# nomadkaraoke/python-audio-separator

Measured on AMD Instinct MI355X. Metric: audio-sec separated / wall-sec (RTF), UVR-MDX-NET 44.1kHz stereo, 1/2/4/8 GPU, higher is better.
Workload: dtype f32 (I/O and accumulators; matrix products on the 16-bit pipe from block-scaled two-part fp16 operands, 22-bit products -- see arithmetic; fp32-exact setting timed in arithmetic_ab)

## Files before the change

### python-audio-separator_amd/csrc/asx.hip

```cpp
#include <hip/hip_runtime.h>

#include <algorithm>
#include <atomic>
#include <cmath>
#include <cstdarg>
#include <cstdio>
#include <cstdlib>
#include <cstring>
#include <functional>
#include <map>
#include <string>
#include <mutex>
#include <vector>

#include "../../include/asx.h"
#include "knobs.h"
#include "resample_plan.h"

static void grant_lds(const void *kernel, int bytes) {
  static std::mutex mu;
  static std::map<const void *, int> granted;
  std::lock_guard<std::mutex> lock(mu);
  int &g = granted[kernel];
  if (bytes > g) {
// ... 31 lines not shown
#include "engine_mdx.h"

static int opt_nonneg(int32_t v) { return v < 0 ? 0 : (int)v; }
static int opt_onoff(int32_t v) { return v > 0 ? 1 : 0; }

static const struct EngineOption {
  const char *key;
  int asx_engine::*field;
  int EngineKnobs::*knob;
  int (*norm)(int32_t);
  const char *refusal = nullptr;
  int shipped = 0;
} kOptions[] = {
    {"winograd", &asx_engine::winograd, &EngineKnobs::winograd, opt_nonneg,
     "asx_set_option: winograd = %d names a superseded kernel generation that only an experimental build carries "
     "(python build.py --experimental); this library has 0 (direct kernel) and 3 (the default)", 3},
    {"winograd_stationary", &asx_engine::winos, &EngineKnobs::winos, opt_nonneg,
     "asx_set_option: the weight-stationary Winograd kernel (measured slower) is in experimental builds only (python build.py --experimental)"},
    {"winograd_bf16x6", &asx_engine::wino6, &EngineKnobs::wino6, opt_nonneg},
    {"gemm_bf16x6", &asx_engine::gemm_bf16x6, &EngineKnobs::gemm_bf16x6, opt_onoff},
    {"gemm_f16x3", &asx_engine::gemm_f16x3, &EngineKnobs::gemm_f16x3, opt_onoff},
    {"conv_direct_f16x3", &asx_engine::conv3h, &EngineKnobs::conv3h, opt_nonneg},
    {"conv_fuse_input", &asx_engine::conv_fuse_input, &EngineKnobs::conv_fuse_input, opt_onoff},
    {"conv_down_bf16x6", &asx_engine::down6, &EngineKnobs::down6, opt_onoff},
    {"conv_up_bf16x6", &asx_engine::up6, &EngineKnobs::up6, opt_onoff},
    {"gemm_pair_images", &asx_engine::pair_images, &EngineKnobs::pair_images, opt_onoff,
     "asx_set_option: gemm_pair_images = 1 needs an experimental build (python build.py --experimental): the pair-image reader measured no "
     "faster in the nets and is not in the default library"},
};

static const EngineOption *find_option(const char *fn, const char *key) {
  for (const EngineOption &o : kOptions)
    if (!strcmp(key, o.key)) return &o;
  set_err("%s: unknown option '%s'", fn, key);
  return nullptr;
}

extern "C" {

int asx_abi_version(void) { return ASX_ABI_VERSION; }
const char *asx_last_error(void) { return g_err; }

int asx_device_count(void) {
  int n = 0;
  if (hipGetDeviceCount(&n) != hipSuccess) return 0;
  return n;
// ... 163 lines not shown
  e->sinc_tab.release();
  for (RsTable *t : e->rs_tabs) {
    t->tab.release();
    delete t;
  }
  e->rs_tabs.clear();
  e->d_window.release();
  e->d_tw.release();
  e->d_env.release();
  e->d_tw3.release();
  e->d_hann3.release();
  e->seam3.release();
  e->d_zeros.release();
  free_conv(e->first);
  free_conv(e->final_);
  for (auto &b : e->enc) free_block(b);
  for (auto &b : e->dec) free_block(b);
  free_block(e->mid);
  for (auto &c : e->ds) free_conv(c);
  for (auto &c : e->us) free_conv(c);
  e->spec_in.release();
  e->spec_out.release();
  for (auto &r : e->R) r.release();
  e->H.release();
  e->frames.release();
  e->chunk_out.release();
  e->d_starts.release();
  e->d_nact.release();
  e->d_peak.release();
  e->d_demixed.release();
  e->d_div.release();
  for (DevBuf *b : {&e->pool_wave, &e->pool_nsong, &e->pool_songs, &e->pool_div, &e->pool_peak}) b->release();
  for (auto &sk : e->skip) sk.release();
  if (e->v3) v3_destroy(e->v3);
  if (e->rof) rof_destroy(e->rof);
  hd_drop_clones(e);
  if (e->ht) ht_destroy(e->ht);
  if (e->hd) hd_destroy(e->hd);
  if (e->vr) vr_destroy(e->vr);
  if (e->ens) ens_destroy(e->ens);
  delete e;
}

int asx_net_begin(asx_engine *e, const asx_net_config *cfg) {
  w3_flush(e);
  REQUIRE(e && cfg, "asx_net_begin: null argument");
// ... 912 lines not shown
    kind = CK_DOWN;
    to = t / 2;
    fo = f / 2;
  } else if (!strcmp(op, "conv1x1")) kind = CK_1X1;
  else if (!strcmp(op, "up")) {
    kind = CK_UP;
    to = 2 * t;
    fo = 2 * f;
    REQUIRE(aux_host, "asx_op_conv(up): skip tensor required");
  } else {
    set_err("asx_op_conv: unknown op '%s'", op);
    return ASX_ERR_INVALID;
  }
  ConvLayer L;
  DevBuf dx, dy, dskip;
  BufGuard g{{&dx, &dy, &dskip, &L.w, &L.b, &L.wu, &L.wu2, &L.wu3, &L.wus, &L.wu6, &L.wu6h, &L.w3h, &L.wd6, &L.wup6}};
  CHK(conv_setup(L, kind, cin, cout, relu ? 1 : 0));
  CHK(conv_pack(L, w_host, b_host, e->winograd));
  CHK(to_dev(dx, x_host, (size_t)B * cin * t * f));
  const size_t ny = (size_t)B * cout * to * fo;
  CHK(dy.ensure(ny * 4));
  HIPCHK(hipMemset(dy.p, 0xff, ny * 4));
  if (kind == CK_UP) CHK(to_dev(dskip, aux_host, ny));
  CHK(conv_launch(e, L, dx.f(), dskip.f(), dy.f(), B, t, f, nullptr));
  CHK(to_host(y_host, dy, ny));
  return ASX_OK;
}

int asx_op_tdf(asx_engine *e, const float *x_host, int32_t B, int32_t c, int32_t t, int32_t k, const float *w_host,
               const float *bias_host, int32_t n, const float *scale_host, const float *shift_host,
               const float *res_host, float *y_host) {
  REQUIRE(e && x_host && w_host && scale_host && shift_host && y_host && B > 0 && c > 0 && t > 0 && k > 0 && n > 0,
          "asx_op_tdf: bad argument");
  HIPCHK(hipSetDevice(e->device));
  TdfLayer L;
  DevBuf dx, dy, dres;
  BufGuard g{{&dx, &dy, &dres, &L.w, &L.bias, &L.scale, &L.shift}};
  CHK(tdf_pack(L, n, k, c, w_host, bias_host, scale_host, shift_host));
  const int64_t M = (int64_t)B * c * t;
  CHK(to_dev(dx, x_host, (size_t)M * k));
  CHK(dy.ensure((size_t)M * n * 4));
  HIPCHK(hipMemset(dy.p, 0xff, (size_t)M * n * 4));
  if (res_host) CHK(to_dev(dres, res_host, (size_t)M * n));
  const int rc = tdf_launch(e, L, dx.f(), res_host ? dres.f() : nullptr, dy.f(), M, t, nullptr);
  const int rc2 = rc == ASX_OK ? to_host(y_host, dy, (size_t)M * n) : rc;
  w3_drop(e, L.w.p);
// ... 1258 lines not shown
```

### python-audio-separator_amd/csrc/engine_core.h

```cpp
#pragma once

static thread_local char g_err[512] = "";
static void set_err(const char *fmt, ...) {
  va_list ap;
  va_start(ap, fmt);
  vsnprintf(g_err, sizeof(g_err), fmt, ap);
  va_end(ap);
}
#define HIPCHK(x)                                                                       \
  do {                                                                                  \
    hipError_t e_ = (x);                                                                \
    if (e_ != hipSuccess) {                                                             \
      set_err("%s:%d %s -> %s", __FILE__, __LINE__, #x, hipGetErrorString(e_));         \
      return ASX_ERR_HIP;                                                               \
    }                                                                                   \
  } while (0)
#define CHK(x)                    \
  do {                            \
    int r_ = (x);                 \
    if (r_ != ASX_OK) return r_;  \
  } while (0)
#define REQUIRE(cond, ...)        \
  do {                            \
    if (!(cond)) {                \
// ... 143 lines not shown
  std::vector<HdNet *> hd_cl;
  DevBuf hd_lstm_ws;
  VrNet *vr = nullptr;
  EnsCtx *ens = nullptr;
  asx_mdx_config cfg{};
  FftPlan plan{};
  DevBuf d_window, d_tw, d_env;
  std::vector<float> custom_window;
  DevBuf d_hann3;
  DevBuf d_tw3, seam3;
  bool fft3 = false;
  bool fft3p = false;
  DevBuf d_zeros;
  bool net_begun = false, net_ready = false;
  asx_net_config net{};
  std::map<std::string, std::vector<float>> host_tensors;
  ConvLayer first, final_;
  std::vector<Block> enc, dec;
  Block mid;
  std::vector<ConvLayer> ds, us;
  int ws_batch = 0;
  DevBuf spec_in, spec_out, R[3], H, HE, frames, chunk_out, d_starts, d_nact, d_peak, d_demixed;
  DevBuf pool_wave, pool_nsong, pool_songs, pool_div, pool_peak;
  DevBuf gn_part;
  DevBuf d_div;
  DivKey div_key;
  DevBuf sinc_tab;
  std::vector<RsTable *> rs_tabs;
  std::mutex rs_mu;
  hipEvent_t div_ev = nullptr;
  hipStream_t div_stream = nullptr;
  std::vector<DevBuf> skip;
  int winograd = 3;
  int winos = 0;
  int gemm_bf16x6 = 1;
  int gemm_f16x3 = 1;
  int wino6 = 144;
  int conv3h = 144;
  int conv_fuse_input = 1;
  int down6 = 1;
  int up6 = 1;
  int pair_images = 0;
  std::vector<W3Entry> w3;
  std::mutex w3_mu;
  bool prof = false;
  int prof_nprod = 0;
  std::vector<ProfRec> recs;
};

static int pick_batch(const asx_engine *e) { return e->cfg.max_batch > 0 ? e->cfg.max_batch : 64; }

#include "batching.h"

template <class F>
static int timed(asx_engine *e, int cls, double flops, double bytes, hipStream_t s, F &&launch) {
  if (!e->prof) {
    launch();
    HIPCHK(hipGetLastError());
    return ASX_OK;
  }
  ProfRec r;
// ... 66 lines not shown
```

### python-audio-separator_amd/csrc/engine_mdx.h

```cpp
#pragma once

template <class CFG>
static void launch_conv_t(const ConvArgs &a, int nblk, hipStream_t s) {
  grant_lds(&conv_mfma_kernel<CFG>, CFG::LDS_BYTES);
  hipLaunchKernelGGL(conv_mfma_kernel<CFG>, dim3(nblk), dim3(256), CFG::LDS_BYTES, s, a);
}

static int conv_tile_h(int kind) { return kind == CK_UP ? 4 : 8; }

static int pick_nrep_conv(int cout) {
  const int ct = (cout + 15) / 16;
  int best = 1, best_pad = 1 << 30;
  for (int n = 3; n >= 1; --n) {
    const int pad = ((ct + n - 1) / n) * n - ct;
    if (pad < best_pad) {
      best_pad = pad;
      best = n;
    }
  }
  return best;
}
static int pick_nrep_up(int cout) {
  const int ct = (cout + 15) / 16;
  if (knobs().up_nrep == 4 && (4 * ct) % 4 == 0) return 4;
// ... 194 lines not shown
static std::atomic<long long> g_down6_launches{0};
static std::atomic<long long> g_up6_launches{0};

struct ConvView {
  int64_t x_bstride = 0;
  int64_t y_bstride = 0;
  const float *res = nullptr;
  int64_t aux_bstride = 0;
  int act = -1;
  float alpha = 1.f;
  const ConvLayer *fin = nullptr;
  const float *fin_x = nullptr;
};

static bool conv3h_takes(const asx_engine *e, const ConvLayer &L, bool dma, const float *res, int act, int T, int F, int64_t y_bstride, const float *y) {
#ifdef ASX_EXPERIMENTAL_KERNELS
  if (e->winos == 1 && L.wus.p != nullptr) return false;
#endif
  return L.kind == CK_3X3 && e->winograd == 3 && e->gemm_bf16x6 > 0 && e->gemm_f16x3 > 0 && e->conv3h > 0 && L.cin <= e->conv3h && L.w3h.p != nullptr && dma &&
         res == nullptr && (act == ACT_RELU || act == ACT_NONE) && F % 32 == 0 && (int64_t)Conv3hCfg::C * T * F < ((int64_t)1 << 29) &&
         y_bstride % 4 == 0 && (reinterpret_cast<uintptr_t>(y) & 15) == 0;
}

static int conv_launch(asx_engine *e, const ConvLayer &L, const float *x, const float *skip, float *y, int B, int T,
                       int F, hipStream_t s, const ConvView &v = ConvView()) {
  ConvArgs a{};
  a.x = x;
  a.wp = L.w.f();
  a.bias = L.b.f();
  a.skip = skip;
  a.res = v.res;
  a.zeros = e->d_zeros.f();
  a.y = y;
  a.B = B;
  a.Cin = L.cin;
  a.Cout = L.cout;
  a.T = T;
  a.F = F;
  a.act = v.act >= 0 ? v.act : (L.relu ? ACT_RELU : ACT_NONE);
  a.alpha = v.alpha;
  REQUIRE(a.act != ACT_ELU || L.kind == CK_1X1, "ELU epilogue: 1x1 convolutions only");
  a.CG = L.cg;
  a.NCI = L.nci;
  a.nt = knobs().nt & 1;
  int cls = ASX_PROF_CONV3X3;
  double taps = 9;
// ... 70 lines not shown
    if (ragged) return k12 ? gos(&conv_winos_kernel<12, 0, true>, WinoSCfg<12>::LDS_BYTES) : gos(&conv_winos_kernel<24, 0, true>, WinoSCfg<24>::LDS_BYTES);
    return k12 ? gos(&conv_winos_kernel<12, 0, false>, WinoSCfg<12>::LDS_BYTES) : gos(&conv_winos_kernel<24, 0, false>, WinoSCfg<24>::LDS_BYTES);
  }
#endif
  if (conv3h_takes(e, L, dma, v.res, a.act, T, F, a.y_bstride, y)) {
    const int nb = L.cin / Conv3hCfg::C;
    const int tilesT = (T + 3) / 4, tilesF = F / 32;
    int bw = 32;
    double best = 1e30;
    for (int cand : {32, 16, 8}) {
      if ((tilesT * cand) % 32 != 0) continue;
      const int tps = tilesT * cand / 32;
      const int bands = (tilesF + cand - 1) / cand, items = B * bands;
      const double cost = (double)(bands * cand) / tilesF * (tps + 1.0) / tps * (double)((items + 7) / 8) / (items / 8.0);
      if (cost < best - 1e-9) {
        best = cost;
        bw = cand;
      }
    }
    if (best > 1e29) bw = 32;
    grant_lds(&conv3h_kernel<0, false>, Conv3hCfg::LDS_BYTES);
    grant_lds(&conv3h_kernel<0, true>, Conv3hCfg::LDS_BYTES);
    grant_lds(&conv3h_kernel<0, false, true>, Conv3hCfg::LDS_BYTES);
    const int64_t plane = (int64_t)T * F;
    return timed(e, cls, flops, bytes, s, [&]() {
      e->prof_nprod = 3;
      for (int ob = 0; ob < nb; ++ob)
        for (int ib = 0; ib < nb; ++ib) {
          Conv3hArgs ca{};
          ca.x = x + (int64_t)ib * Conv3hCfg::C * plane;
          ca.y = y + (int64_t)ob * Conv3hCfg::C * plane;
          ca.prev = ib > 0 ? ca.y : nullptr;
          ca.wimg = reinterpret_cast<const u32x4 *>(reinterpret_cast<const uint32_t *>(L.w3h.p) + (size_t)(ob * nb + ib) * Conv3hCfg::IMG_U32);
          ca.bias = ib == 0 ? L.b.f() + ob * Conv3hCfg::C : nullptr;
          ca.B = B;
          ca.T = T;
          ca.F = F;
          ca.x_bstride = a.x_bstride;
          ca.y_bstride = a.y_bstride;
          ca.act = ib == nb - 1 ? a.act : ACT_NONE;
          ca.tilesT = tilesT;
          ca.tilesF = tilesF;
          ca.bw = bw;
          ca.tps = (tilesT * bw) % 32 == 0 ? tilesT * bw / 32 : tilesT;
          if (v.fin) {
            ca.xin = v.fin_x;
            ca.xin_bstride = 4 * plane;
            ca.w1 = v.fin->w1f.f();
            hipLaunchKernelGGL((conv3h_kernel<0, false, true>), dim3(256), dim3(512), Conv3hCfg::LDS_BYTES, s, ca);
            g_conv3h_fin_launches.fetch_add(1);
          } else if (ib > 0) hipLaunchKernelGGL((conv3h_kernel<0, true>), dim3(256), dim3(512), Conv3hCfg::LDS_BYTES, s, ca);
          else hipLaunchKernelGGL((conv3h_kernel<0, false>), dim3(256), dim3(512), Conv3hCfg::LDS_BYTES, s, ca);
          g_conv3h_launches.fetch_add(1);
        }
    });
  }
  if (L.kind == CK_3X3 && e->winograd == 3 && e->gemm_bf16x6 > 0 && e->wino6 > 0 && L.cin >= e->wino6 && dma && L.wu6_nci > 0 &&
      (int64_t)T * F < ((int64_t)1 << 24)) {
    ConvArgs wa = a;
    const bool h3 = e->gemm_f16x3 > 0 && L.wu6h.p != nullptr;
    wa.wp = reinterpret_cast<const float *>(h3 ? L.wu6h.p : L.wu6.p);
    wa.CG = L.wu_cg;
    wa.NCI = L.wu6_nci;
    wa.tilesT = (a.To + Wino6Cfg::TH - 1) / Wino6Cfg::TH;
    wa.tilesF = (a.Fo + Wino6Cfg::TW - 1) / Wino6Cfg::TW;
    const int64_t S = (int64_t)wa.tilesT * wa.tilesF * B;
    const int64_t nb = ((S + 7) / 8) * 8 * wa.CG;
    if (nb < ((int64_t)1 << 31)) {
      grant_lds(&conv_wino6_kernel<0, 1>, Wino6Cfg::LDS_BYTES);
      grant_lds(&conv_wino6_kernel<0, 1, true>, Wino6Cfg::LDS_BYTES);
      g_wino6_launches.fetch_add(1);
      if (h3) g_wino6h_launches.fetch_add(1);
      return timed(e, cls, flops, bytes, s, [&]() {
        e->prof_nprod = h3 ? 3 : 6;
// ... 776 lines not shown
  CHK(conv_launch(e, e->final_, cur, nullptr, spec_out, B, T, F, s));
  return ASX_OK;
}

static int ensure_workspace(asx_engine *e, int Bchunks, bool need_net) {
  const int T = e->cfg.segment_size, Fq = e->cfg.dim_f;
  const int mult = (need_net && e->cfg.enable_denoise) ? 2 : 1;
  const size_t Bn = (size_t)Bchunks * mult;
  CHK(e->spec_in.ensure(Bn * 4 * T * Fq * 4));
  CHK(e->frames.ensure((size_t)Bchunks * 2 * T * e->cfg.n_fft * 4));
  if (need_net) {
    CHK(e->spec_out.ensure(Bn * 4 * T * Fq * 4));
    const size_t lvl0 = Bn * e->net.g * T * Fq * 4;
    for (int i = 0; i < 3; ++i) CHK(e->R[i].ensure(lvl0));
    CHK(e->H.ensure(Bn * e->net.g * T * (Fq / std::max(1, e->net.bn)) * 4 + 256));
    CHK(e->HE.ensure(Bn * e->net.g * T * (size_t)((Fq / std::max(1, e->net.bn) + 127) / 128) * 4 + 256));
    if (e->net.norm == 1) CHK(e->gn_part.ensure(Bn * (size_t)e->net.g * (e->net.num_blocks / 2 + 1) * 16));
    const int n = e->net.num_blocks / 2;
    e->skip.resize(n);
    for (int i = 0; i < n; ++i) {
      const size_t c = (size_t)e->net.g * (i + 1), t = T >> i, f = Fq >> i;
      CHK(e->skip[i].ensure(Bn * c * t * f * 4));
    }
  }
  e->ws_batch = std::max(e->ws_batch, Bchunks);
  return ASX_OK;
}
```

### python-audio-separator_amd/csrc/engine_v3.h

```cpp
#pragma once
#include "v3_norm.h"

struct V3Norm {
  DevBuf g, b;
  int c = 0;
};

struct V3Block {
  int in_c = 0, c = 0, f = 0;
  V3Norm n_tfc1, n_tdf0, n_tdf1, n_tfc2;
  ConvLayer tfc1, tfc2, shortcut;
  TdfLayer tdf0, tdf1;
};

struct V3Net {
  asx_v3_config cfg{};
  float act_alpha = 1.f;
  bool begun = false, ready = false;
  ConvLayer first, final0, final1;
  std::vector<std::vector<V3Block>> enc, dec;
  std::vector<V3Block> mid;
  std::vector<ConvLayer> ds, us;
  std::vector<V3Norm> ds_n, us_n;
  int ws_batch = 0;
// ... 181 lines not shown
  const int64_t P0 = (int64_t)T * Fs;
  const int c0 = cf.num_channels_model;
  const size_t big = (size_t)B * 2 * c0 * P0 * 4;
  CHK(n.cat0.ensure((size_t)B * (dim_c + c0) * P0 * 4));
  CHK(n.firstout.ensure((size_t)B * c0 * P0 * 4));
  CHK(n.A.ensure(big));
  CHK(n.S.ensure(big / 2));
  CHK(n.X1.ensure(big / 2));
  CHK(n.X2.ensure(big / 2));
  CHK(n.XB.ensure(big / 2));
  CHK(n.CUR.ensure(big / 2));
  CHK(n.H.ensure(big / 2 / cf.bottleneck_factor + 256));
  CHK(n.HA.ensure(big / 2 / cf.bottleneck_factor + 256));
  int cmax = c0 + cf.growth * cf.num_scales;
  CHK(n.stats.ensure((size_t)B * 2 * cmax * sizeof(float2)));
  if (cf.norm > V3_NORM_GROUP) CHK(n.gn_part.ensure((size_t)B * v3_norm_groups(cf.norm) * V3_GN_MAX_SPLIT * sizeof(double2)));
  n.lvl.resize(cf.num_scales);
  int c = c0;
  int64_t P = P0;
  for (int i = 0; i < cf.num_scales; ++i) {
    CHK(n.lvl[i].ensure((size_t)B * 2 * c * P * 4));
    c += cf.growth;
    P /= 4;
  }
  CHK(n.out_spec.ensure((size_t)B * cf.num_targets * dim_c * P0 * 4));
  CHK(n.frames.ensure((size_t)B * cf.num_targets * 2 * T * e->cfg.n_fft * 4));
  n.ws_batch = B;
  return ASX_OK;
}

static int v3_core_dev(asx_engine *e, int B, hipStream_t s) {
  V3Net &n = *e->v3;
  const asx_v3_config &cf = n.cfg;
  const int T = e->cfg.segment_size, k = cf.num_subbands, Fs = e->cfg.dim_f / k;
  const int dim_c = k * cf.num_channels * 2;
  const int c0 = cf.num_channels_model;
  const int64_t P0 = (int64_t)T * Fs;
  const int64_t cat_bs = (int64_t)(dim_c + c0) * P0;
  {
    ConvView v;
    v.x_bstride = cat_bs;
    CHK(conv_launch(e, n.first, n.cat0.f(), nullptr, n.firstout.f(), B, T, Fs, s, v));
  }
  V3View x{n.firstout.f(), (int64_t)c0 * P0};
  int c = c0, t = T, f = Fs;
  for (int i = 0; i < cf.num_scales; ++i) {
// ... 138 lines not shown
```

### python-audio-separator_amd/csrc/kernels_conv3h.h

```cpp
#pragma once
#include <cstring>
#include <vector>

#include "kernels_gemm3.h"

namespace asx {

struct Conv3hArgs {
  const float *x;
  float *y;
  const u32x4 *wimg;
  const float *bias;
  int B, T, F;
  int64_t x_bstride, y_bstride;
  int act;
  int tilesT, tilesF;
  int bw, tps;
  const float *prev;
  long long *dbg;
  const float *xin;
  const float *w1;
  int64_t xin_bstride;
};

struct Conv3hCfg {
  static constexpr int C = 48, CG8 = C / 8;
  static constexpr int TH = 4, TW = 32, IW = TW + 2;
  static constexpr int PSTR = C * 2;
  static constexpr int ROWB = IW * PSTR;
  static constexpr int RING = 12;
  static constexpr int PART = RING * ROWB;
  static constexpr int KGY = 3 * CG8;
  static constexpr int SPK = (KGY + 3) / 4;
  static constexpr int NST = (3 * KGY + 3) / 4;
  static constexpr int WKY = (KGY / 4) * 3 * 2 * 1024 + 3 * 2 * 512;
  static constexpr int WBYTES = 3 * WKY;
  static constexpr int W_OFF = 0, X_OFF = WBYTES, TAB_OFF = X_OFF + 2 * PART;
  static constexpr int LDS_BYTES = TAB_OFF + 64;
  static constexpr size_t IMG_U32 = WBYTES / 4 + 48;
  static constexpr int EUP = 8;

  enum { FULL = 0, MERGED = 1, PADDED = 2 };
  struct Stage {
    int kind, ky, kyb, sg;
    int rfrom, rto;
  };
  static constexpr int NPROG = 2;
  static constexpr int PROG_OF_WAVE[4] = {0, 1, 0, 0};
  static constexpr Stage PLAN[NPROG][NST] = {
      {{FULL, 0, 0, 0, -1, -1}, {FULL, 0, 0, 1, -1, -1}, {FULL, 0, 0, 2, -1, -1}, {FULL, 0, 0, 3, -1, -1},
       {FULL, 1, 1, 0, -1, -1}, {FULL, 1, 1, 1, -1, -1}, {FULL, 1, 1, 2, -1, -1}, {FULL, 1, 1, 3, -1, -1},
       {MERGED, 0, 1, 4, 1, 2},
       {FULL, 2, 2, 0, -1, -1}, {FULL, 2, 2, 1, -1, -1}, {FULL, 2, 2, 2, -1, -1}, {FULL, 2, 2, 3, -1, -1},
       {PADDED, 2, 2, 4, -1, -1}},
      {{FULL, 0, 0, 0, -1, -1}, {FULL, 0, 0, 1, -1, -1}, {FULL, 0, 0, 2, -1, -1}, {FULL, 0, 0, 3, -1, -1},
       {PADDED, 0, 0, 4, 0, 1},
       {FULL, 1, 1, 0, -1, -1}, {FULL, 1, 1, 1, -1, -1}, {FULL, 1, 1, 2, -1, -1}, {FULL, 1, 1, 3, -1, -1},
       {FULL, 2, 2, 0, -1, -1}, {FULL, 2, 2, 1, -1, -1}, {FULL, 2, 2, 2, -1, -1}, {FULL, 2, 2, 3, -1, -1},
       {MERGED, 1, 2, 4, -1, -1}}};
  static constexpr Stage plan_find(int p, int kind) {
    for (int s = 0; s < NST; ++s)
      if (PLAN[p][s].kind == kind) return PLAN[p][s];
    return Stage{-1, -1, -1, -1, -1, -1};
// ... 129 lines not shown
  unsigned hh = 0, ll = 0;
  asm("v_fma_mixlo_f16 %0, %1, %2, 0 op_sel_hi:[0,0,0]" : "+v"(hh) : "v"(x0), "v"(s));
  asm("v_fma_mixhi_f16 %0, %1, %2, 0 op_sel_hi:[0,0,0]" : "+v"(hh) : "v"(x1), "v"(s));
  asm("v_fma_mixlo_f16 %0, %1, %2, -%3 op_sel:[0,0,0] op_sel_hi:[0,0,1]" : "+v"(ll) : "v"(x0), "v"(s), "v"(hh));
  asm("v_fma_mixhi_f16 %0, %1, %2, -%3 op_sel:[0,0,1] op_sel_hi:[0,0,1]" : "+v"(ll) : "v"(x1), "v"(s), "v"(hh));
  h = hh;
  l = ll;
}

template <int BM>
__device__ __forceinline__ float ror8m(float keep, float from) {
  return __builtin_bit_cast(float, __builtin_amdgcn_update_dpp(__builtin_bit_cast(int, keep), __builtin_bit_cast(int, from), 0x128, 0xf, BM, false));
}

template <bool FIN>
struct Conv3hFinRegs {};
template <>
struct Conv3hFinRegs<true> {
  f32x4 rin[4][4];
  bool ok[4];
  float w1[8][4], b1[8];
};

template <int ABL = 0, bool ACC = false, bool FIN = false>
__global__ __launch_bounds__(512) __attribute__((amdgpu_waves_per_eu(2, 2))) void conv3h_kernel(Conv3hArgs a) {
  using CFG = Conv3hCfg;
  extern __shared__ float lds_f[];
  char *lds = reinterpret_cast<char *>(lds_f);
  const int tid = threadIdx.x;
  const int lane = tid & 63;
  const int wave = __builtin_amdgcn_readfirstlane(tid >> 6);
  const int wg = blockIdx.x;
  float *maxtab = reinterpret_cast<float *>(lds + CFG::TAB_OFF);
  int *exps = reinterpret_cast<int *>(lds + CFG::TAB_OFF + 32);

  {
    const u32x4 *src = a.wimg;
    u32x4 *dst = reinterpret_cast<u32x4 *>(lds + CFG::W_OFF);
    for (int i = tid; i < CFG::WBYTES / 16; i += 512) dst[i] = src[i];
  }
  const int64_t TF = (int64_t)a.T * a.F;
  const int NB = conv3h_nblocks(a, wg);
  const int row0 = conv3h_row0(a, wg);
  const unsigned plane_bytes = (unsigned)(CFG::C * TF * 4);

  if (wave >= 4) {
    const int ptid = tid - 256, pw = wave - 4;
    int row, cig, q;
    if (ptid < 160) {
// ... 167 lines not shown
    constexpr CFG::Stage MST = CFG::plan_find(PROG, CFG::MERGED), PST = CFG::plan_find(PROG, CFG::PADDED);
    const int li = lane & 15, g = lane >> 4;
    int vl[CFG::SPK];
#pragma unroll
    for (int sg = 0; sg < CFG::SPK; ++sg) {
      int kk = 4 * sg + g;
      kk = kk < CFG::KGY ? kk : CFG::KGY - 2 + (g & 1);
      vl[sg] = (kk / CFG::CG8 + li) * CFG::PSTR + (kk % CFG::CG8) * 16 + CFG::X_OFF;
    }
    const char *wl = lds + CFG::W_OFF + lane * 16;
    const bool pad_lane = g >= (CFG::KGY % 4);
    int whp[3][2], whm[3][2];
#pragma unroll
    for (int c = 0; c < 3; ++c)
#pragma unroll
      for (int p = 0; p < 2; ++p) {
        const int hf = CFG::W_OFF + (CFG::SPK - 1) * 6144 + (c * 2 + p) * 512 + (lane & 31) * 16;
        whp[c][p] = pad_lane ? CFG::TAB_OFF + 48 : hf + PST.ky * CFG::WKY;
        whm[c][p] = hf + (pad_lane ? MST.kyb : MST.ky) * CFG::WKY;
      }
    if (tid < 4) reinterpret_cast<unsigned *>(lds + CFG::TAB_OFF + 48)[tid] = 0u;
    const int *wexp = reinterpret_cast<const int *>(a.wimg) + CFG::WBYTES / 4;
    int ew[3];
    float bz[3];
#pragma unroll
    for (int c = 0; c < 3; ++c) {
      ew[c] = wexp[c * 16 + li];
      bz[c] = a.bias ? a.bias[c * 16 + li] : 0.f;
    }
    f32x4 pend[6];
    int pend_vo = 0;
    __amdgpu_buffer_rsrc_t pend_rs = __builtin_amdgcn_make_buffer_rsrc(a.y, 0, 0, 0x00020000);
    int soff[6];
#pragma unroll
    for (int k = 0; k < 6; ++k) soff[k] = (int)(((k / 2) * 16 + (k % 2) * 8) * TF * 4);
    const bool hi8 = (li & 8) != 0;
    const float act_lo = a.act == ACT_RELU ? 0.f : -__builtin_inff();

    auto flush_one = [&](auto kc) {
      constexpr int K = decltype(kc)::value;
      if constexpr ((ABL & 4) == 0) {
        __builtin_amdgcn_raw_buffer_store_b128(__builtin_bit_cast(u32x4, pend[K]), pend_rs, pend_vo, soff[K], (ABL & 512) ? 0 : 2);
      } else {
        if (pend[K].x == 1.2345e-30f) a.y[0] = pend[K].y;
      }
    };
    f32x4 pacc[2][3];
    int pend_e = 0;
    f32x4 pprev[6];
#pragma unroll
    for (int k = 0; k < 6; ++k) pprev[k] = (f32x4){0.f, 0.f, 0.f, 0.f};
    auto epi_chunk = [&](auto kc) {
      constexpr int K = decltype(kc)::value, c = K / 2;
      const float sc = __builtin_ldexpf(1.0f, -(pend_e + ew[c]));
      f32x4 v[2];
#pragma unroll
      for (int qq = 0; qq < 2; ++qq) {
        v[qq].x = __builtin_fmaf(pacc[qq][c].x, sc, bz[c]);
        v[qq].y = __builtin_fmaf(pacc[qq][c].y, sc, bz[c]);
        v[qq].z = __builtin_fmaf(pacc[qq][c].z, sc, bz[c]);
        v[qq].w = __builtin_fmaf(pacc[qq][c].w, sc, bz[c]);
      }
      f32x4 o;
      if constexpr (K % 2 == 0) o = (f32x4){ror8m<0xC>(v[0].x, v[1].x), ror8m<0xC>(v[0].y, v[1].y), ror8m<0xC>(v[0].z, v[1].z), ror8m<0xC>(v[0].w, v[1].w)};
      else o = (f32x4){ror8m<0x3>(v[1].x, v[0].x), ror8m<0x3>(v[1].y, v[0].y), ror8m<0x3>(v[1].z, v[0].z), ror8m<0x3>(v[1].w, v[0].w)};
      if constexpr (ACC) o += pprev[K];
      pend[K] = (f32x4){fmaxf(o.x, act_lo), fmaxf(o.y, act_lo), fmaxf(o.z, act_lo), fmaxf(o.w, act_lo)};
    };
    auto flush = [&]() {
      epi_chunk(IntC<0>{});
      epi_chunk(IntC<1>{});
      epi_chunk(IntC<2>{});
      epi_chunk(IntC<3>{});
      epi_chunk(IntC<4>{});
      epi_chunk(IntC<5>{});
      flush_one(IntC<0>{});
      flush_one(IntC<1>{});
      flush_one(IntC<2>{});
      flush_one(IntC<3>{});
      flush_one(IntC<4>{});
      flush_one(IntC<5>{});
      pend_rs = __builtin_amdgcn_make_buffer_rsrc(a.y, 0, 0, 0x00020000);
    };

    __syncthreads();
    __syncthreads();
    Conv3hWalk wk;
    conv3h_walk_init(a, wg, wk);
    int s3 = 0;
    for (int s = 0; s < NB; ++s) {
      const int tb = wk.b, j = wk.j, f0 = wk.strip * 32;
      conv3h_walk_next(a, wg, wk);
      if constexpr ((ABL & 32) != 0) {
        if (wg == 0 && wave == 0 && s < 64) {
          const long long t = __builtin_amdgcn_s_memtime();
          if (lane == 0) a.dbg[s * 8 + 4] = t;
        }
      }
      if (j >= 0) {
        const int tt = row0 + j * 4 + wave;
        const bool cur_ok = tt < a.T && f0 < a.F;
        const int cur_vo = (((li & 7) * a.T + tt) * a.F + f0 + ((li >> 3) * 4 + g) * 4) * 4;
        const int sp = s3 == 0 ? 2 : s3 - 1;
        const int e_cur = __builtin_amdgcn_readfirstlane(exps[s3]), e_old = __builtin_amdgcn_readfirstlane(exps[sp]);
        int rowoff[3], eky[3];
#pragma unroll
        for (int ky = 0; ky < 3; ++ky) {
          const int u = wave + ky;
          rowoff[ky] = (u < 2 ? sp * 4 + 2 + u : s3 * 4 + u - 2) * CFG::ROWB;
          eky[ky] = u < 2 ? e_old : e_cur;
        }
        const int xm = (pad_lane ? rowoff[MST.kyb] : rowoff[MST.ky]) + vl[CFG::SPK - 1];
        f32x4 acc[2][3];
#pragma unroll
        for (int p = 0; p < 2; ++p)
#pragma unroll
          for (int c = 0; c < 3; ++c) acc[p][c] = (f32x4){0.f, 0.f, 0.f, 0.f};
        constexpr int PF = (ABL & 2048) ? 2 : 1;
        f16x8 wf[PF + 1][3][2], xf[PF + 1][2][2];
        auto load_stage = [&](auto bufc, auto sc) {
          constexpr int BUF = decltype(bufc)::value, S = decltype(sc)::value;
          constexpr CFG::Stage ST = CFG::PLAN[PROG][S];
          constexpr int KY = ST.ky, SG = ST.sg;
#pragma unroll
          for (int c = 0; c < 3; ++c)
// ... 26 lines not shown
#pragma unroll
            for (int c = 0; c < 3; ++c) acc[qq][c] = ASX_MFMA_F16(xf[BUF][qq][0], wf[BUF][c][0], acc[qq][c]);
        };
        __builtin_amdgcn_sched_barrier(0);
        load_stage(IntC<0>{}, IntC<0>{});
        if constexpr (PF == 2) load_stage(IntC<1>{}, IntC<1>{});
        __builtin_amdgcn_sched_barrier(0);
        auto run = [&](auto sc, auto &&self) {
          constexpr int S = decltype(sc)::value;
          if constexpr (S + PF < CFG::NST) load_stage(IntC<(S + PF) % (PF + 1)>{}, IntC<S + PF>{});
          mfma_stage(IntC<S % (PF + 1)>{});
          constexpr bool EPI = (ABL & 128) == 0 && S >= 1 && S <= 6;
          if constexpr (EPI) epi_chunk(IntC<S - 1>{});
          if constexpr (S + PF < CFG::NST) {
#pragma unroll
            for (int i = 0; i < 9; ++i) {
              __builtin_amdgcn_sched_group_barrier(0x100, 1, 0);
              __builtin_amdgcn_sched_group_barrier(0x008, 2, 0);
              if constexpr (EPI) __builtin_amdgcn_sched_group_barrier(0x002, 2, 0);
            }
            __builtin_amdgcn_sched_group_barrier(0x100, 1, 0);
          }
          __builtin_amdgcn_sched_barrier(0);
          if constexpr (ACC && S == 7) {
            __amdgpu_buffer_rsrc_t prs = __builtin_amdgcn_make_buffer_rsrc(const_cast<float *>(a.prev + (int64_t)tb * a.y_bstride), 0, cur_ok ? plane_bytes : 0u, 0x00020000);
#pragma unroll
            for (int k = 0; k < 6; ++k) pprev[k] = __builtin_bit_cast(f32x4, __builtin_amdgcn_raw_buffer_load_b128(prs, cur_vo, soff[k], 0));
            __builtin_amdgcn_sched_barrier(0);
          }
          if constexpr ((ABL & 128) == 0 && S >= 8 && S <= 13) {
            flush_one(IntC<S - 8>{});
            if constexpr (S == 13) pend_rs = __builtin_amdgcn_make_buffer_rsrc(a.y, 0, 0, 0x00020000);
            __builtin_amdgcn_sched_barrier(0);
          }
          if constexpr ((ABL & 256) == 0 && CFG::PLAN[PROG][S].rto >= 0) {
            const int d = eky[CFG::PLAN[PROG][S].rto] - eky[CFG::PLAN[PROG][S].rfrom];
            if (d != 0) {
#pragma unroll
              for (int qq = 0; qq < 2; ++qq)
#pragma unroll
                for (int c = 0; c < 3; ++c) {
                  acc[qq][c].x = __builtin_ldexpf(acc[qq][c].x, d);
                  acc[qq][c].y = __builtin_ldexpf(acc[qq][c].y, d);
                  acc[qq][c].z = __builtin_ldexpf(acc[qq][c].z, d);
                  acc[qq][c].w = __builtin_ldexpf(acc[qq][c].w, d);
                }
            }
            __builtin_amdgcn_sched_barrier(0);
          }
          if constexpr (S + 1 < CFG::NST) self(IntC<S + 1>{}, self);
        };
        run(IntC<0>{}, run);
        if constexpr ((ABL & 32) != 0) {
          if (wg == 0 && wave == 0 && s < 64) {
            const long long t = __builtin_amdgcn_s_memtime();
            if (lane == 0) a.dbg[s * 8 + 5] = t;
          }
        }
#pragma unroll
        for (int qq = 0; qq < 2; ++qq)
#pragma unroll
          for (int c = 0; c < 3; ++c) pacc[qq][c] = acc[qq][c];
        pend_e = e_cur;
        pend_rs = __builtin_amdgcn_make_buffer_rsrc(a.y + (int64_t)tb * a.y_bstride, 0, cur_ok ? plane_bytes : 0u, 0x00020000);
        pend_vo = cur_vo;
        if constexpr ((ABL & 128) != 0) flush();
      } else {
        flush();
      }
      if constexpr ((ABL & 32) != 0) {
        if (wg == 0 && wave == 0 && s < 64) {
          const long long t = __builtin_amdgcn_s_memtime();
          if (lane == 0) a.dbg[s * 8 + 6] = t;
        }
      }
      __syncthreads();
      s3 = s3 == 2 ? 0 : s3 + 1;
    }
    flush();
    };
    static_assert(CFG::NPROG == 2 && CFG::PROG_OF_WAVE[0] == 0 && CFG::PROG_OF_WAVE[1] == 1 && CFG::PROG_OF_WAVE[2] == 0 && CFG::PROG_OF_WAVE[3] == 0, "the branch below is the table");
    if (wave == 1) consume(IntC<1>{});
    else consume(IntC<0>{});
  }
}

}
```

### python-audio-separator_amd/csrc/knobs.h

```cpp
#pragma once

#include <algorithm>
#include <climits>
#include <cstdint>
#include <cstdlib>

#ifndef ASX_TDF2_DEFAULT
#define ASX_TDF2_DEFAULT 1
#endif

constexpr int HD_MAX_GROUPS = 6;

namespace knob {
inline bool set(const char *name) { return getenv(name) != nullptr; }
inline int num(const char *name, int def) { return set(name) ? atoi(getenv(name)) : def; }
inline int64_t num64(const char *name, int64_t def) { return set(name) ? atoll(getenv(name)) : def; }
inline double real(const char *name, double def) { return set(name) ? atof(getenv(name)) : def; }
inline bool on_unless_0(const char *name) { return !(set(name) && atoi(getenv(name)) == 0); }
inline bool off_unless_nonzero(const char *name) { return set(name) && atoi(getenv(name)) != 0; }
inline int clamped(const char *name, int def, int lo, int hi = INT_MAX) { return set(name) ? std::max(lo, std::min(hi, atoi(getenv(name)))) : def; }
}

struct Knobs {
  int poison = knob::num("ASX_POISON", -1);
// ... 58 lines not shown
  bool rof_fuse = knob::on_unless_0("ASX_ROF_FUSE");
};

inline const Knobs &knobs() {
  static const Knobs k;
  return k;
}

struct EngineKnobs {
#ifdef ASX_EXPERIMENTAL_KERNELS
  int winograd = knob::clamped("ASX_WINOGRAD", 3, 0);
  int winos = knob::clamped("ASX_WINOS", 0, 0);
  int pair_images = knob::num("ASX_PAIR_IMAGES", 0);
#else
  int winograd = knob::num("ASX_WINOGRAD", 3) <= 0 ? 0 : 3;
  int winos = 0;
  int pair_images = 0;
#endif
  int gemm_bf16x6 = knob::num("ASX_GEMM_BF16X6", 1);
  int gemm_f16x3 = knob::num("ASX_GEMM_F16X3", 1);
  int wino6 = knob::clamped("ASX_WINO6", 144, 0);
  int conv3h = knob::clamped("ASX_CONV3H", 144, 0);
  int conv_fuse_input = 1;
  int down6 = knob::num("ASX_DOWN6", 1);
  int up6 = knob::num("ASX_UP6", 1);
  bool fft3 = knob::on_unless_0("ASX_FFT3");
  bool fft3p = knob::on_unless_0("ASX_FFT3P");
};
```

Before: 1650.

## Carry conv3h input-block partial sums through a lane-ordered scratch buffer

When a 3x3 f16x3 conv spans several input-channel blocks, intermediate partial sums are now written to and read back from a dedicated scratch buffer. The buffer is stored in the kernel's per-wave register order, so each step does contiguous 128-bit stores and loads and skips the permute shuffles and strided planar reads of the old accumulate-into-y path. Only the last input block applies the activation and writes the planar output. The cost is a workspace allocation sized per layer, plus three more kernel template variants to compile and grant LDS for.

```diff
diff --git a/python-audio-separator_amd/csrc/asx.hip b/python-audio-separator_amd/csrc/asx.hip
--- a/python-audio-separator_amd/csrc/asx.hip
+++ b/python-audio-separator_amd/csrc/asx.hip
@@ -77,6 +77,7 @@
     {"gemm_f16x3", &asx_engine::gemm_f16x3, &EngineKnobs::gemm_f16x3, opt_onoff},
     {"conv_direct_f16x3", &asx_engine::conv3h, &EngineKnobs::conv3h, opt_nonneg},
     {"conv_fuse_input", &asx_engine::conv_fuse_input, &EngineKnobs::conv_fuse_input, opt_onoff},
+    {"conv3h_partial_scratch", &asx_engine::conv3h_ps, &EngineKnobs::conv3h_ps, opt_onoff},
     {"conv_down_bf16x6", &asx_engine::down6, &EngineKnobs::down6, opt_onoff},
     {"conv_up_bf16x6", &asx_engine::up6, &EngineKnobs::up6, opt_onoff},
     {"gemm_pair_images", &asx_engine::pair_images, &EngineKnobs::pair_images, opt_onoff,
@@ -286,6 +287,7 @@
   e->spec_in.release();
   e->spec_out.release();
   for (auto &r : e->R) r.release();
+  e->c3h_ps.release();
   e->H.release();
   e->frames.release();
   e->chunk_out.release();
@@ -1244,6 +1246,7 @@
   CHK(dy.ensure(ny * 4));
   HIPCHK(hipMemset(dy.p, 0xff, ny * 4));
   if (kind == CK_UP) CHK(to_dev(dskip, aux_host, ny));
+  CHK(e->c3h_ps.ensure(conv3h_ps_need(L, B, t, f)));
   CHK(conv_launch(e, L, dx.f(), dskip.f(), dy.f(), B, t, f, nullptr));
   CHK(to_host(y_host, dy, ny));
   return ASX_OK;
diff --git a/python-audio-separator_amd/csrc/engine_core.h b/python-audio-separator_amd/csrc/engine_core.h
--- a/python-audio-separator_amd/csrc/engine_core.h
+++ b/python-audio-separator_amd/csrc/engine_core.h
@@ -189,6 +189,7 @@
   int ws_batch = 0;
   DevBuf spec_in, spec_out, R[3], H, HE, frames, chunk_out, d_starts, d_nact, d_peak, d_demixed;
   DevBuf pool_wave, pool_nsong, pool_songs, pool_div, pool_peak;
+  DevBuf c3h_ps;
   DevBuf gn_part;
   DevBuf d_div;
   DivKey div_key;
@@ -204,6 +205,7 @@
   int gemm_f16x3 = 1;
   int wino6 = 144;
   int conv3h = 144;
+  int conv3h_ps = 1;
   int conv_fuse_input = 1;
   int down6 = 1;
   int up6 = 1;
diff --git a/python-audio-separator_amd/csrc/engine_mdx.h b/python-audio-separator_amd/csrc/engine_mdx.h
--- a/python-audio-separator_amd/csrc/engine_mdx.h
+++ b/python-audio-separator_amd/csrc/engine_mdx.h
@@ -240,6 +240,11 @@
          y_bstride % 4 == 0 && (reinterpret_cast<uintptr_t>(y) & 15) == 0;
 }
 
+static size_t conv3h_ps_need(const ConvLayer &L, int B, int T, int F) {
+  if (L.kind != CK_3X3 || L.w3h.p == nullptr || L.cin <= Conv3hCfg::C || F % 32 != 0 || B <= 0 || T <= 0) return 0;
+  return (size_t)Conv3hCfg::ps_bytes(B, (T + 3) / 4, F / 32);
+}
+
 static int conv_launch(asx_engine *e, const ConvLayer &L, const float *x, const float *skip, float *y, int B, int T,
                        int F, hipStream_t s, const ConvView &v = ConvView()) {
   ConvArgs a{};
@@ -356,34 +361,47 @@
     grant_lds(&conv3h_kernel<0, false>, Conv3hCfg::LDS_BYTES);
     grant_lds(&conv3h_kernel<0, true>, Conv3hCfg::LDS_BYTES);
     grant_lds(&conv3h_kernel<0, false, true>, Conv3hCfg::LDS_BYTES);
+    grant_lds(&conv3h_kernel<0, false, false, 1>, Conv3hCfg::LDS_BYTES);
+    grant_lds(&conv3h_kernel<0, false, false, 2>, Conv3hCfg::LDS_BYTES);
+    grant_lds(&conv3h_kernel<0, false, false, 3>, Conv3hCfg::LDS_BYTES);
     const int64_t plane = (int64_t)T * F;
+    const bool ps = e->conv3h_ps > 0 && nb > 1;
+    const int64_t ps_item = Conv3hCfg::ps_item_bytes(tilesT, tilesF);
+    REQUIRE(!ps || (ps_item < ((int64_t)1 << 32) && e->c3h_ps.p != nullptr && e->c3h_ps.bytes >= conv3h_ps_need(L, B, T, F)),
+            "conv3h_kernel: the partial-sum scratch is not sized for %d x %d x %d (the workspace set-up sizes it)", B, T, F);
+    Conv3hArgs walk{};
+    walk.B = B;
+    walk.T = T;
+    walk.F = F;
+    walk.x_bstride = a.x_bstride;
+    walk.y_bstride = a.y_bstride;
+    walk.tilesT = tilesT;
+    walk.tilesF = tilesF;
+    walk.bw = bw;
+    walk.tps = (tilesT * bw) % 32 == 0 ? tilesT * bw / 32 : tilesT;
+    walk.ps = ps ? e->c3h_ps.p : nullptr;
+    walk.ps_bstride = ps_item;
     return timed(e, cls, flops, bytes, s, [&]() {
       e->prof_nprod = 3;
       for (int ob = 0; ob < nb; ++ob)
         for (int ib = 0; ib < nb; ++ib) {
-          Conv3hArgs ca{};
+          Conv3hArgs ca = walk;
           ca.x = x + (int64_t)ib * Conv3hCfg::C * plane;
           ca.y = y + (int64_t)ob * Conv3hCfg::C * plane;
-          ca.prev = ib > 0 ? ca.y : nullptr;
+          ca.prev = ib > 0 && !ps ? ca.y : nullptr;
           ca.wimg = reinterpret_cast<const u32x4 *>(reinterpret_cast<const uint32_t *>(L.w3h.p) + (size_t)(ob * nb + ib) * Conv3hCfg::IMG_U32);
           ca.bias = ib == 0 ? L.b.f() + ob * Conv3hCfg::C : nullptr;
-          ca.B = B;
-          ca.T = T;
-          ca.F = F;
-          ca.x_bstride = a.x_bstride;
-          ca.y_bstride = a.y_bstride;
           ca.act = ib == nb - 1 ? a.act : ACT_NONE;
-          ca.tilesT = tilesT;
-          ca.tilesF = tilesF;
-          ca.bw = bw;
-          ca.tps = (tilesT * bw) % 32 == 0 ? tilesT * bw / 32 : tilesT;
           if (v.fin) {
             ca.xin = v.fin_x;
             ca.xin_bstride = 4 * plane;
             ca.w1 = v.fin->w1f.f();
             hipLaunchKernelGGL((conv3h_kernel<0, false, true>), dim3(256), dim3(512), Conv3hCfg::LDS_BYTES, s, ca);
             g_conv3h_fin_launches.fetch_add(1);
-          } else if (ib > 0) hipLaunchKernelGGL((conv3h_kernel<0, true>), dim3(256), dim3(512), Conv3hCfg::LDS_BYTES, s, ca);
+          } else if (ps && ib == 0) hipLaunchKernelGGL((conv3h_kernel<0, false, false, 2>), dim3(256), dim3(512), Conv3hCfg::LDS_BYTES, s, ca);
+          else if (ps && ib < nb - 1) hipLaunchKernelGGL((conv3h_kernel<0, false, false, 3>), dim3(256), dim3(512), Conv3hCfg::LDS_BYTES, s, ca);
+          else if (ps) hipLaunchKernelGGL((conv3h_kernel<0, false, false, 1>), dim3(256), dim3(512), Conv3hCfg::LDS_BYTES, s, ca);
+          else if (ib > 0) hipLaunchKernelGGL((conv3h_kernel<0, true>), dim3(256), dim3(512), Conv3hCfg::LDS_BYTES, s, ca);
           else hipLaunchKernelGGL((conv3h_kernel<0, false>), dim3(256), dim3(512), Conv3hCfg::LDS_BYTES, s, ca);
           g_conv3h_launches.fetch_add(1);
         }
@@ -1206,6 +1224,14 @@
       const size_t c = (size_t)e->net.g * (i + 1), t = T >> i, f = Fq >> i;
       CHK(e->skip[i].ensure(Bn * c * t * f * 4));
     }
+    size_t ps = 0;
+    auto ps_block = [&](const Block &blk) {
+      for (const ConvLayer &L : blk.tfc) ps = std::max(ps, conv3h_ps_need(L, (int)Bn, blk.t, blk.f));
+    };
+    for (const Block &blk : e->enc) ps_block(blk);
+    ps_block(e->mid);
+    for (const Block &blk : e->dec) ps_block(blk);
+    CHK(e->c3h_ps.ensure(ps));
   }
   e->ws_batch = std::max(e->ws_batch, Bchunks);
   return ASX_OK;
diff --git a/python-audio-separator_amd/csrc/engine_v3.h b/python-audio-separator_amd/csrc/engine_v3.h
--- a/python-audio-separator_amd/csrc/engine_v3.h
+++ b/python-audio-separator_amd/csrc/engine_v3.h
@@ -227,6 +227,19 @@
     CHK(n.lvl[i].ensure((size_t)B * 2 * c * P * 4));
     c += cf.growth;
     P /= 4;
+  }
+  {
+    size_t ps = 0;
+    auto ps_blocks = [&](const std::vector<V3Block> &bs, int t, int f) {
+      for (const V3Block &b : bs) ps = std::max(ps, std::max(conv3h_ps_need(b.tfc1, B, t, f), conv3h_ps_need(b.tfc2, B, t, f)));
+    };
+    int t = T, f = Fs;
+    for (int i = 0; i < cf.num_scales; ++i, t /= 2, f /= 2) {
+      ps_blocks(n.enc[i], t, f);
+      ps_blocks(n.dec[cf.num_scales - 1 - i], t, f);
+    }
+    ps_blocks(n.mid, t, f);
+    CHK(e->c3h_ps.ensure(ps));
   }
   CHK(n.out_spec.ensure((size_t)B * cf.num_targets * dim_c * P0 * 4));
   CHK(n.frames.ensure((size_t)B * cf.num_targets * 2 * T * e->cfg.n_fft * 4));
diff --git a/python-audio-separator_amd/csrc/kernels_conv3h.h b/python-audio-separator_amd/csrc/kernels_conv3h.h
--- a/python-audio-separator_amd/csrc/kernels_conv3h.h
+++ b/python-audio-separator_amd/csrc/kernels_conv3h.h
@@ -21,6 +21,8 @@
   const float *xin;
   const float *w1;
   int64_t xin_bstride;
+  void *ps;
+  int64_t ps_bstride;
 };
 
 struct Conv3hCfg {
@@ -39,6 +41,14 @@
   static constexpr int LDS_BYTES = TAB_OFF + 64;
   static constexpr size_t IMG_U32 = WBYTES / 4 + 48;
   static constexpr int EUP = 8;
+
+  static constexpr int PS_STORE = 1024, PS_WAVE = 6 * PS_STORE, PS_TILE = 4 * PS_WAVE;
+  static constexpr int64_t ps_item_bytes(int tilesT, int tilesF) { return (int64_t)tilesF * tilesT * PS_TILE; }
+  static constexpr int64_t ps_bytes(int B, int tilesT, int tilesF) { return (int64_t)B * ps_item_bytes(tilesT, tilesF); }
+  static constexpr unsigned ps_wave_off(int tilesT, int strip, int jt, int r) { return (unsigned)((strip * tilesT + jt) * 4 + r) * (unsigned)PS_WAVE; }
+  static constexpr int64_t ps_off(int tilesT, int tilesF, int b, int strip, int jt, int r, int k, int lane) {
+    return (int64_t)b * ps_item_bytes(tilesT, tilesF) + ps_wave_off(tilesT, strip, jt, r) + k * PS_STORE + lane * 16;
+  }
 
   enum { FULL = 0, MERGED = 1, PADDED = 2 };
   struct Stage {
@@ -214,9 +224,11 @@
   float w1[8][4], b1[8];
 };
 
-template <int ABL = 0, bool ACC = false, bool FIN = false>
+template <int ABL = 0, bool ACC = false, bool FIN = false, int PS = 0>
 __global__ __launch_bounds__(512) __attribute__((amdgpu_waves_per_eu(2, 2))) void conv3h_kernel(Conv3hArgs a) {
   using CFG = Conv3hCfg;
+  constexpr bool PIN = (PS & 1) != 0, POUT = (PS & 2) != 0;
+  static_assert(!(PS != 0 && (ACC || FIN)), "partial sums through the scratch: neither the planar accumulate mode nor the fused input");
   extern __shared__ float lds_f[];
   char *lds = reinterpret_cast<char *>(lds_f);
   const int tid = threadIdx.x;
@@ -430,10 +442,11 @@
     if (tid < 4) reinterpret_cast<unsigned *>(lds + CFG::TAB_OFF + 48)[tid] = 0u;
     const int *wexp = reinterpret_cast<const int *>(a.wimg) + CFG::WBYTES / 4;
     int ew[3];
-    float bz[3];
+    float bz[3], wsc[3];
 #pragma unroll
     for (int c = 0; c < 3; ++c) {
       ew[c] = wexp[c * 16 + li];
+      wsc[c] = __builtin_ldexpf(1.0f, -ew[c]);
       bz[c] = a.bias ? a.bias[c * 16 + li] : 0.f;
     }
     f32x4 pend[6];
@@ -442,13 +455,14 @@
     int soff[6];
 #pragma unroll
     for (int k = 0; k < 6; ++k) soff[k] = (int)(((k / 2) * 16 + (k % 2) * 8) * TF * 4);
-    const bool hi8 = (li & 8) != 0;
-    const float act_lo = a.act == ACT_RELU ? 0.f : -__builtin_inff();
+    const unsigned ps_item = (unsigned)CFG::ps_item_bytes(a.tilesT, a.tilesF);
+    const float act_lo = !POUT && a.act == ACT_RELU ? 0.f : -__builtin_inff();
 
     auto flush_one = [&](auto kc) {
       constexpr int K = decltype(kc)::value;
       if constexpr ((ABL & 4) == 0) {
-        __builtin_amdgcn_raw_buffer_store_b128(__builtin_bit_cast(u32x4, pend[K]), pend_rs, pend_vo, soff[K], (ABL & 512) ? 0 : 2);
+        if constexpr (POUT) __builtin_amdgcn_raw_buffer_store_b128(__builtin_bit_cast(u32x4, pend[K]), pend_rs, lane * 16, pend_vo + K * CFG::PS_STORE, (ABL & 512) ? 0 : 2);
+        else __builtin_amdgcn_raw_buffer_store_b128(__builtin_bit_cast(u32x4, pend[K]), pend_rs, pend_vo, soff[K], (ABL & 512) ? 0 : 2);
       } else {
         if (pend[K].x == 1.2345e-30f) a.y[0] = pend[K].y;
       }
@@ -460,7 +474,15 @@
     for (int k = 0; k < 6; ++k) pprev[k] = (f32x4){0.f, 0.f, 0.f, 0.f};
     auto epi_chunk = [&](auto kc) {
       constexpr int K = decltype(kc)::value, c = K / 2;
-      const float sc = __builtin_ldexpf(1.0f, -(pend_e + ew[c]));
+      const float sc = PS != 0 ? __builtin_ldexpf(wsc[c], -pend_e) : __builtin_ldexpf(1.0f, -(pend_e + ew[c]));
+      if constexpr (POUT) {
+        constexpr int qq = K % 2;
+        f32x4 o = (f32x4){__builtin_fmaf(pacc[qq][c].x, sc, bz[c]), __builtin_fmaf(pacc[qq][c].y, sc, bz[c]), __builtin_fmaf(pacc[qq][c].z, sc, bz[c]),
+                          __builtin_fmaf(pacc[qq][c].w, sc, bz[c])};
+        if constexpr (PIN) o += pprev[K];
+        pend[K] = (f32x4){fmaxf(o.x, act_lo), fmaxf(o.y, act_lo), fmaxf(o.z, act_lo), fmaxf(o.w, act_lo)};
+        return;
+      }
       f32x4 v[2];
 #pragma unroll
       for (int qq = 0; qq < 2; ++qq) {
@@ -468,6 +490,7 @@
         v[qq].y = __builtin_fmaf(pacc[qq][c].y, sc, bz[c]);
         v[qq].z = __builtin_fmaf(pacc[qq][c].z, sc, bz[c]);
         v[qq].w = __builtin_fmaf(pacc[qq][c].w, sc, bz[c]);
+        if constexpr (PIN) v[qq] += pprev[c * 2 + qq];
       }
       f32x4 o;
       if constexpr (K % 2 == 0) o = (f32x4){ror8m<0xC>(v[0].x, v[1].x), ror8m<0xC>(v[0].y, v[1].y), ror8m<0xC>(v[0].z, v[1].z), ror8m<0xC>(v[0].w, v[1].w)};
@@ -497,7 +520,7 @@
     conv3h_walk_init(a, wg, wk);
     int s3 = 0;
     for (int s = 0; s < NB; ++s) {
-      const int tb = wk.b, j = wk.j, f0 = wk.strip * 32;
+      const int tb = wk.b, j = wk.j, wk_strip = wk.strip, f0 = wk_strip * 32;
       conv3h_walk_next(a, wg, wk);
       if constexpr ((ABL & 32) != 0) {
         if (wg == 0 && wave == 0 && s < 64) {
@@ -509,6 +532,7 @@
         const int tt = row0 + j * 4 + wave;
         const bool cur_ok = tt < a.T && f0 < a.F;
         const int cur_vo = (((li & 7) * a.T + tt) * a.F + f0 + ((li >> 3) * 4 + g) * 4) * 4;
+        const int cur_ps = (int)CFG::ps_wave_off(a.tilesT, wk_strip, (row0 >> 2) + j, wave);
         const int sp = s3 == 0 ? 2 : s3 - 1;
         const int e_cur = __builtin_amdgcn_readfirstlane(exps[s3]), e_old = __builtin_amdgcn_readfirstlane(exps[sp]);
         int rowoff[3], eky[3];
@@ -581,6 +605,12 @@
             __builtin_amdgcn_sched_group_barrier(0x100, 1, 0);
           }
           __builtin_amdgcn_sched_barrier(0);
+          if constexpr (PIN && S == 7) {
+            __amdgpu_buffer_rsrc_t prs = __builtin_amdgcn_make_buffer_rsrc(static_cast<char *>(a.ps) + (int64_t)tb * a.ps_bstride, 0, cur_ok ? ps_item : 0u, 0x00020000);
+#pragma unroll
+            for (int k = 0; k < 6; ++k) pprev[k] = __builtin_bit_cast(f32x4, __builtin_amdgcn_raw_buffer_load_b128(prs, lane * 16, cur_ps + k * CFG::PS_STORE, 0));
+            __builtin_amdgcn_sched_barrier(0);
+          }
           if constexpr (ACC && S == 7) {
             __amdgpu_buffer_rsrc_t prs = __builtin_amdgcn_make_buffer_rsrc(const_cast<float *>(a.prev + (int64_t)tb * a.y_bstride), 0, cur_ok ? plane_bytes : 0u, 0x00020000);
 #pragma unroll
@@ -621,8 +651,13 @@
 #pragma unroll
           for (int c = 0; c < 3; ++c) pacc[qq][c] = acc[qq][c];
         pend_e = e_cur;
-        pend_rs = __builtin_amdgcn_make_buffer_rsrc(a.y + (int64_t)tb * a.y_bstride, 0, cur_ok ? plane_bytes : 0u, 0x00020000);
-        pend_vo = cur_vo;
+        if constexpr (POUT) {
+          pend_rs = __builtin_amdgcn_make_buffer_rsrc(static_cast<char *>(a.ps) + (int64_t)tb * a.ps_bstride, 0, cur_ok ? ps_item : 0u, 0x00020000);
+          pend_vo = cur_ps;
+        } else {
+          pend_rs = __builtin_amdgcn_make_buffer_rsrc(a.y + (int64_t)tb * a.y_bstride, 0, cur_ok ? plane_bytes : 0u, 0x00020000);
+          pend_vo = cur_vo;
+        }
         if constexpr ((ABL & 128) != 0) flush();
       } else {
         flush();
diff --git a/python-audio-separator_amd/csrc/knobs.h b/python-audio-separator_amd/csrc/knobs.h
--- a/python-audio-separator_amd/csrc/knobs.h
+++ b/python-audio-separator_amd/csrc/knobs.h
@@ -104,6 +104,7 @@
   int wino6 = knob::clamped("ASX_WINO6", 144, 0);
   int conv3h = knob::clamped("ASX_CONV3H", 144, 0);
   int conv_fuse_input = 1;
+  int conv3h_ps = 1;
   int down6 = knob::num("ASX_DOWN6", 1);
   int up6 = knob::num("ASX_UP6", 1);
   bool fft3 = knob::on_unless_0("ASX_FFT3");
```

After: 1686, median of 6. 1.02x the previous value.
